# XThomasBU/video-gen-evals

Hardware: AMD Instinct MI355X
Metric: videos/sec scored (AC+TC) @32 frames/clip, 1/2/4/8 MI355X; |Δscore| vs ref (higher is better)
Workload: dtype f32x3; 1 GPU; BASELINE config 2: fusion-encoder fwd + AC/TC metrics, 256 clips x 32 frames per GPU, pre-extracted features resident in HBM (featurise included in the step); clips_per_gpu=256, frames_per_clip=32, windows_per_encode=256, parallelism=video-sharded x1

## Files before the change

video-gen-evals_amd/csrc/vge_encoder_x3s.hip:

```cpp
#include "vge_x3.h"
#include <type_traits>

#ifdef VGE_TRACE
__device__ long long g_x3s_trace[64 * 8 * 128];
#define XTS(k)                                                                                                       \
  do {                                                                                                              \
    if (tr_on && blockIdx.x < 64 && (threadIdx.x & 63) == 0)                                                        \
      g_x3s_trace[(blockIdx.x * 8 + (threadIdx.x >> 6)) * 128 + (k)] = __builtin_amdgcn_s_memtime();                 \
  } while (0)
#else
#define XTS(k) \
  do {         \
  } while (0)
#endif

namespace {

using vge::EncDescX3;

#ifndef X3S_TRACE_ROUND
#define X3S_TRACE_ROUND 0
#endif
#ifndef X3S_GELU
#define X3S_GELU 1
#endif
#ifndef X3S_PRIO
#define X3S_PRIO 1
#endif
constexpr int X3S_WMAX = 4;
#ifndef X3S_PF_QUAD
#define X3S_PF_QUAD 4
#endif
#ifndef X3S_PF_PAIR
#define X3S_PF_PAIR 8
#endif
#ifndef X3S_PF16_QUAD
#define X3S_PF16_QUAD 8
#endif
#ifndef X3S_PF16_PAIR
#define X3S_PF16_PAIR 8
#endif
#ifndef X3S_ROT
#define X3S_ROT 0
#endif
#ifndef X3S_SKIP
#define X3S_SKIP 1
#endif
constexpr int XR = 536;
constexpr int XRB = 2 * XR;
constexpr int XLO = 528;
template <int W>
constexpr int x3s_g() { return 32 / W; }
template <int W>
constexpr int x3s_wsb() { return 32 * XRB + (W >= 4 ? 128 : 0); }
template <int W>
constexpr int x3s_zr() { return W * x3s_wsb<W>(); }
template <int W>
__host__ __device__ constexpr int x3s_rwin(int r) { return ((r & 3) + 8 * (r >> 2)) / x3s_g<W>(); }
template <int W>
__host__ __device__ constexpr int x3s_rfr0(int t, int r) {
  return x3s_g<W>() * t + ((r & 3) + 8 * (r >> 2)) % x3s_g<W>();
}
template <int W, bool SKIP>
__device__ __forceinline__ bool x3s_tap_ok(int t, int o) {
  constexpr int G = x3s_g<W>();
  return !(X3S_SKIP && SKIP) || (G * t + G - 1 + o >= 0 && G * t + o <= 31);
}
constexpr int X3S_AUX_OFF = (x3s_zr<X3S_WMAX>() + XRB + 15) / 16 * 16;

struct X3sAux {
  int rexp[2][32 * X3S_WMAX];
  float stats[2][X3S_WMAX][8][2];
  float mx[2][2][X3S_WMAX][4];
  int ex[2][2][X3S_WMAX];
  int cnt[2];
};
constexpr int X3S_PRE_WAVE = 32 * 64 + 256;
constexpr int X3S_PRE_OFF = (X3S_AUX_OFF + (int)sizeof(X3sAux) + 15) / 16 * 16;
constexpr int X3S_LDS_BYTES = X3S_PRE_OFF + 8 * X3S_PRE_WAVE;
static_assert(X3S_AUX_OFF % 16 == 0, "aux alignment");
static_assert(X3S_LDS_BYTES <= 160 * 1024, "LDS");

template <int W, bool SKIP, bool SP>
__device__ __forceinline__ void stream_part(Acc<W, 1>& acc, const char* wb, int ntap, unsigned loff, const char* xa,
                                            int i, int dil, int ctr, int rot) {
  constexpr int R = W, G = x3s_g<W>();
  constexpr int PF = SP ? (R >= 4 ? X3S_PF_QUAD : X3S_PF_PAIR) : (R >= 4 ? X3S_PF16_QUAD : X3S_PF16_PAIR);
  static_assert(8 % PF == 0, "ring depth must divide a tap's 8 chunks");
  const char* xw = xa + (i / G) * x3s_wsb<W>();
  const int fi = i % G;
  const char* xz = xa + x3s_zr<W>();
  auto rowp = [&](int k, int t) -> const char* {
    const int tt = G * t + fi + (k - ctr) * dil;
    return (unsigned)tt < 32u ? xw + tt * XRB : xz;
  };
  const __amdgpu_buffer_rsrc_t rs =
      __builtin_amdgcn_make_buffer_rsrc(const_cast<char*>(wb), (short)0, 0x7FFFFFF0, 0x00020000);
  const unsigned loff_l = loff + PLANE_B;
  auto ldb = [&](int k, int j, BFrag<1>& b) {
    const int so = (k * 16 + ((j + rot) & 7)) * CHUNK_B;
    b.h[0] = __builtin_bit_cast(half8, __builtin_amdgcn_raw_buffer_load_b128(rs, loff, so, 0));
    if constexpr (SP) b.l[0] = __builtin_bit_cast(half8, __builtin_amdgcn_raw_buffer_load_b128(rs, loff_l, so, 0));
  };
  BFrag<1> b[PF];
#pragma unroll
  for (int j = 0; j < PF - 1; ++j) ldb(0, j, b[j]);
  half8 ah[R], al[R];
  const char* pt[R];
  bool okc[R];
#pragma unroll
  for (int t = 0; t < R; ++t) {
    pt[t] = rowp(0, t);
    okc[t] = x3s_tap_ok<W, SKIP>(t, -ctr * dil);
    if (okc[t]) {
      ah[t] = *reinterpret_cast<const half8*>(pt[t] + rot * 32);
      if constexpr (SP) al[t] = *reinterpret_cast<const half8*>(pt[t] + rot * 32 + XLO);
    }
  }
  for (int k = 0; k < ntap; ++k) {
    const bool more = k + 1 < ntap;
    const int kn = more ? k + 1 : k;
    const char* pn[R];
    bool okn[R];
#pragma unroll
    for (int t = 0; t < R; ++t) {
      pn[t] = rowp(kn, t);
      okn[t] = x3s_tap_ok<W, SKIP>(t, (kn - ctr) * dil);
    }
#pragma unroll
    for (int j = 0; j < 8; ++j) {
#if !(VGE_ABL & 2)
      if (j + PF - 1 < 8) ldb(k, j + PF - 1, b[(j + PF - 1) % PF]);
      else ldb(kn, more ? j + PF - 1 - 8 : 7, b[(j + PF - 1) % PF]);
#endif
#pragma unroll
      for (int t = 0; t < R; ++t) {
#if !(VGE_ABL & 1)
        if (okc[t]) {
          acc.c[t][0] = mfma32(ah[t], b[j % PF].h[0], acc.c[t][0]);
          if constexpr (SP) {
            acc.c[t][0] = mfma32(ah[t], b[j % PF].l[0], acc.c[t][0]);
            acc.c[t][0] = mfma32(al[t], b[j % PF].h[0], acc.c[t][0]);
          }
        }
#endif
#if !(VGE_ABL & 4)
        if (j < 7 ? okc[t] : okn[t]) {
          const char* q = j < 7 ? pt[t] + ((j + 1 + rot) & 7) * 32 : pn[t] + rot * 32;
          ah[t] = *reinterpret_cast<const half8*>(q);
          if constexpr (SP) al[t] = *reinterpret_cast<const half8*>(q + XLO);
        }
#endif
        __builtin_amdgcn_sched_barrier(0);
      }
      asm volatile("" ::: "memory");
    }
#pragma unroll
    for (int t = 0; t < R; ++t) {
      pt[t] = pn[t];
      okc[t] = okn[t];
    }
  }
}

__device__ __forceinline__ float gload(const float* p) {
  return *(const __attribute__((address_space(1))) float*)p;
}

template <int W, bool SP>
__device__ __forceinline__ void conv_x3s_body(const float* __restrict__ feats, int n_windows, int win0,
                                              const EncDescX3& ed, int e, float* __restrict__ enc_out, char* lds_raw,
                                              int& n_ex, int* __restrict__ status, int spin_limit,
                                              [[maybe_unused]] bool tr_on) {
  constexpr int R = W, G = x3s_g<W>(), WSB = x3s_wsb<W>();
  _Float16* X = reinterpret_cast<_Float16*>(lds_raw);
  char* Xb = lds_raw;
  X3sAux& ax = *reinterpret_cast<X3sAux*>(lds_raw + X3S_AUX_OFF);

  const int tid = threadIdx.x;
  const int wave = __builtin_amdgcn_readfirstlane(tid >> 6);
  const int grp = wave >> 2, wg = wave & 3;
  int lane, i, h, col;
  unsigned loff;
  const char* xa;
  auto lane_setup = [&]() {
    int t = tid;
    asm volatile("" : "+v"(t));
    lane = t & 63;
    i = lane & 31;
    h = lane >> 5;
    col = wave * 32 + i;
    loff = (unsigned)((h * 256 + col) * 16);
    xa = reinterpret_cast<const char*>(X) + h * 16;
  };
  lane_setup();
  auto crow = [&](int t, int r) { return x3s_rwin<W>(r) * 32 + x3s_rfr0<W>(t, r) + 4 * h; };
  auto cofs = [&](int t, int r) { return x3s_rwin<W>(r) * WSB + x3s_rfr0<W>(t, r) * XRB; };

  Acc<R, 1> acc;
  floatx16 res[R];
  for (int c = tid; c < XR; c += 512)
    *reinterpret_cast<_Float16*>(Xb + x3s_zr<W>() + 2 * c) = (_Float16)0.0f;

  auto afn_stem = [&](int c, AFrag<R>& f) {
#pragma unroll
    for (int t = 0; t < R; ++t) {
      const char* q = xa + (i / G) * WSB + (G * t + i % G) * XRB + c * 32;
      f.h[t] = *reinterpret_cast<const half8*>(q);
      if constexpr (SP) f.l[t] = *reinterpret_cast<const half8*>(q + XLO);
    }
  };
  XTS(0);
  acc.zero();
  constexpr int RPW = 32 * W / 8;
  constexpr int PG = W <= 2 ? 2 : 1;
  for (int p0 = 0; p0 < ed.n_stem_panels; p0 += PG) {
    float a[PG][RPW][4];
#pragma unroll
    for (int q = 0; q < PG; ++q) {
      const int p = p0 + q;
      const int kw = p < ed.n_stem_panels ? min(256, ed.d_in - p * 256) : 0;
#pragma unroll
      for (int jr = 0; jr < RPW; ++jr) {
        const int r = wave * RPW + jr;
        const int w = win0 + (r >> 5);
        const float* src = feats + ((size_t)w * VGE_T + (r & 31)) * ed.ld + ed.in_col + p * 256;
#pragma unroll
        for (int jc = 0; jc < 4; ++jc) {
          const int c = lane + 64 * jc;
          a[q][jr][jc] = (c < kw && w < n_windows) ? gload(src + c) : 0.f;
        }
      }
    }
#pragma unroll
    for (int q = 0; q < PG; ++q) {
      const int p = p0 + q;
      if (p >= ed.n_stem_panels) break;
      const int kw = min(256, ed.d_in - p * 256);
      int* ecur = ax.rexp[p & 1];
#pragma unroll
      for (int jr = 0; jr < RPW; ++jr) {
        float m = fmaxf(fmaxf(fabsf(a[q][jr][0]), fabsf(a[q][jr][1])), fmaxf(fabsf(a[q][jr][2]), fabsf(a[q][jr][3])));
        m = wave_max_all(m);
        const int ex = fp16_range_exp(m);
        const int r = wave * RPW + jr;
        if (lane == 0) ecur[r] = ex;
        _Float16* xr = reinterpret_cast<_Float16*>(Xb + (r >> 5) * WSB + (r & 31) * XRB);
#pragma unroll
        for (int jc = 0; jc < 4; ++jc) {
          const int c = lane + 64 * jc;
          if constexpr (SP) split_store(xr + c, xr + XLO / 2 + c, ldexpf(a[q][jr][jc], -ex));
          else xr[c] = (_Float16)ldexpf(a[q][jr][jc], -ex);
        }
      }
      __syncthreads();
      if (p == 0) XTS(122);
      if (p > 0) {
        const int* eprev = ax.rexp[(p - 1) & 1];
#pragma unroll
        for (int t = 0; t < R; ++t)
#pragma unroll
          for (int r = 0; r < 16; ++r) acc.c[t][0][r] *= ldexpf(1.0f, eprev[crow(t, r)] - ecur[crow(t, r)]);
      }
      run_stream<SP ? CONV_PF : CONV_PF16, SP>(acc, reinterpret_cast<const char*>(ed.stem) + (size_t)p * 16 * CHUNK_B,
                                ((kw + 127) >> 7) * STREAM_GROUP, loff, afn_stem);
      if (p == 0) XTS(123);
      __syncthreads();
    }
  }

  auto group_max = [&](float (&m)[R]) {
    const int par = n_ex & 1;
#pragma unroll
    for (int t = 0; t < R; ++t) {
      const float w = wave_max_last(m[t]);
      if (lane == 63) ax.mx[par][grp][t][wg] = w;
    }
    ++n_ex;
    if (lane == 63) __hip_atomic_fetch_add(&ax.cnt[grp], 1, __ATOMIC_RELEASE, __HIP_MEMORY_SCOPE_WORKGROUP);
    int spin = 0;
    for (; spin < spin_limit && __builtin_amdgcn_readfirstlane(__hip_atomic_load(
                                    &ax.cnt[grp], __ATOMIC_ACQUIRE, __HIP_MEMORY_SCOPE_WORKGROUP)) < 4 * n_ex;
         ++spin)
      __builtin_amdgcn_s_sleep(1);
    if (spin >= spin_limit &&
        __builtin_amdgcn_readfirstlane(__hip_atomic_load(&ax.cnt[grp], __ATOMIC_ACQUIRE, __HIP_MEMORY_SCOPE_WORKGROUP)) <
            4 * n_ex &&
        lane == 0)
      __hip_atomic_store(status, 1, __ATOMIC_RELAXED, __HIP_MEMORY_SCOPE_SYSTEM);
#pragma unroll
    for (int t = 0; t < R; ++t)
      m[t] = fmaxf(fmaxf(ax.mx[par][grp][t][0], ax.mx[par][grp][t][1]),
                   fmaxf(ax.mx[par][grp][t][2], ax.mx[par][grp][t][3]));
  };
  [[maybe_unused]] int tslot = 64;
  auto store_act = [&](auto get, int par) {
    XTS(tslot + 1);
    float m[R];
#pragma unroll
    for (int v = 0; v < R; ++v) m[v] = 0.f;
#pragma unroll
    for (int t = 0; t < R; ++t) {
      const floatx16& x = get(t);
#pragma unroll
      for (int r = 0; r < 16; ++r) m[x3s_rwin<W>(r)] = fmaxf(m[x3s_rwin<W>(r)], fabsf(x[r]));
    }
    group_max(m);
    XTS(tslot + 2);
    float scv[R];
#pragma unroll
    for (int v = 0; v < R; ++v) {
      const int ex = fp16_range_exp(m[v]);
      if (wg == 0 && lane == 0) ax.ex[par][grp][v] = ex;
      scv[v] = ldexpf(1.0f, -ex);
    }
    char* bh = Xb + (4 * h * XR + col) * 2;
#pragma unroll
    for (int t = 0; t < R; ++t) {
      const floatx16& x = get(t);
#pragma unroll
      for (int r = 0; r < 16; ++r) {
        const float y = x[r] * scv[x3s_rwin<W>(r)];
        const _Float16 hi = (_Float16)y;
        const int off = cofs(t, r);
        *reinterpret_cast<_Float16*>(bh + off) = hi;
        if constexpr (SP) *reinterpret_cast<_Float16*>(bh + XLO + off) = (_Float16)(y - (float)hi);
      }
    }
    XTS(tslot + 3);
    tslot += 4;
  };
  auto gn_stats = [&](int b, int t, float& mu, float& rstd) {
    const float(*s)[2] = ax.stats[b & 1][t];
    const float m = (((s[0][0] + s[1][0]) + (s[2][0] + s[3][0])) + ((s[4][0] + s[5][0]) + (s[6][0] + s[7][0]))) * 0.125f;
    float q = 0.f, d = 0.f;
#pragma unroll
    for (int w = 0; w < 8; ++w) {
      q += s[w][1];
      const float dm = s[w][0] - m;
      d = fmaf(dm, dm, d);
    }
    mu = m;
    rstd = 1.0f / sqrtf(fmaf(d, 1024.0f, q) * (1.0f / 8192.0f) + 1e-5f);
  };
  auto gelu_tile = [&](floatx16& v) {
    float y[16];
#pragma unroll
    for (int k = 0; k < 16; ++k) y[k] = v[k];
#if X3S_GELU
    gelu_fast_s(y);
#else
    gelu_many_s(y);
#endif
#pragma unroll
    for (int k = 0; k < 16; ++k) v[k] = y[k];
  };

  auto stem_epilogue = [&]() {
    XTS(tslot);
    const int* efin = ax.rexp[(ed.n_stem_panels - 1) & 1];
    const float wcs = gload(ed.cs + col);
#pragma unroll
    for (int t = 0; t < R; ++t) {
#pragma unroll
      for (int r = 0; r < 16; ++r) res[t][r] = ldexpf(acc.c[t][0][r] * wcs, efin[crow(t, r)]);
    }
    store_act([&](int t) -> const floatx16& { return res[t]; }, 0);
  };

  float pre_wcs = 0.f, pre_sx = 0.f, pre_sy = 0.f;
  char* pre_lds = lds_raw + X3S_PRE_OFF + wave * X3S_PRE_WAVE;
  auto prefetch = [&](auto kind_tag, int gi) {
    constexpr int KIND = decltype(kind_tag)::value;
    const int blk = gi >> 1;
    pre_wcs = gload(ed.cs + (1 + gi) * 256 + col);
    if constexpr (KIND == 2) {
      pre_sx = gload(ed.fold + 3 * 256 * 16 + col * 2);
      pre_sy = gload(ed.fold + 3 * 256 * 16 + col * 2 + 1);
    } else if constexpr (KIND == 0) {
      if (blk > 0) {
        const float* fb = ed.fold + ((size_t)(blk - 1) * 256 + wave * 32) * 16;
        glds16(fb + lane * 4, pre_lds);
        glds16(fb + 256 + lane * 4, pre_lds + 1024);
        const float* gsrc = (h ? ed.gn_b : ed.gn_w) + (blk - 1) * 256 + col;
        __builtin_amdgcn_global_load_lds((const __attribute__((address_space(1))) void*)gsrc,
                                         (__attribute__((address_space(3))) void*)(pre_lds + 2048), 4, 0, 0);
        asm volatile("" ::: "memory");
      }
    }
  };

  auto epilogue = [&](auto kind_tag, int gi) {
    constexpr int KIND = decltype(kind_tag)::value;
    XTS(tslot);
    const int par = gi & 1, blk = gi >> 1;
    const float wcs = pre_wcs;
    float scv[R];
#pragma unroll
    for (int v = 0; v < R; ++v) scv[v] = ldexpf(1.0f, ax.ex[par][1][v]) * wcs;
    if constexpr (KIND == 2) {
      const float2 sp = {pre_sx, pre_sy};
      float* ob = enc_out + (size_t)e * n_windows * VGE_T * VGE_D + col;
#pragma unroll
      for (int v = 0; v < R; ++v) {
        float mu, rstd;
        gn_stats(3, v, mu, rstd);
        const int win = win0 + v;
        if (win < n_windows) {
#pragma unroll
          for (int t = 0; t < R; ++t)
#pragma unroll
            for (int r = 0; r < 16; ++r)
              if (x3s_rwin<W>(r) == v)
                ob[((size_t)win * VGE_T + x3s_rfr0<W>(t, r) + 4 * h) * VGE_D] =
                    fmaf(rstd, fmaf(acc.c[t][0][r], scv[v], -mu * sp.x), sp.y);
        }
      }
    } else {
      constexpr int GH = G / 2;
      float cg[16], cb[16], gsv[R], gshv[R], muv[R], rstdv[R];
      if constexpr (KIND == 0) {
        if (blk > 0) {
          const int dil = 1 << blk;
          vmcnt0();
          const char* pl = pre_lds + i * 64;
          const floatx4 pre_g = *reinterpret_cast<const floatx4*>(pl);
          const float pre_g4 = *reinterpret_cast<const float*>(pl + 16);
          const floatx4 pre_b = *reinterpret_cast<const floatx4*>(pl + 32);
          const float pre_b4 = *reinterpret_cast<const float*>(pl + 48);
          const float pre_gw = *reinterpret_cast<const float*>(pre_lds + 2048 + i * 4);
          const float pre_gb = *reinterpret_cast<const float*>(pre_lds + 2048 + 128 + i * 4);
#pragma unroll
          for (int f = 0; f < 16; ++f) {
            const int row = x3s_rfr0<W>(f / GH, f % GH) + 4 * h;
            const bool k0 = row >= 2 * dil, k1 = row >= dil, k3 = row < 32 - dil, k4 = row < 32 - 2 * dil;
            cg[f] = (((k0 ? pre_g.x : 0.f) + (k1 ? pre_g.y : 0.f)) + pre_g.z) + (k3 ? pre_g.w : 0.f) + (k4 ? pre_g4 : 0.f);
            cb[f] = (((k0 ? pre_b.x : 0.f) + (k1 ? pre_b.y : 0.f)) + pre_b.z) + (k3 ? pre_b.w : 0.f) + (k4 ? pre_b4 : 0.f);
          }
#pragma unroll
          for (int v = 0; v < R; ++v) {
            gn_stats(blk - 1, v, muv[v], rstdv[v]);
            gsv[v] = rstdv[v] * pre_gw;
            gshv[v] = fmaf(-muv[v], gsv[v], pre_gb);
          }
        }
      }
#pragma unroll
      for (int t = 0; t < R; ++t) {
        floatx16& x = acc.c[t][0];
        if constexpr (KIND == 0) {
          if (blk > 0) {
#pragma unroll
            for (int r = 0; r < 16; ++r) {
              const int v = x3s_rwin<W>(r), f = t * GH + r % GH;
              res[t][r] = fmaf(res[t][r], gsv[v], gshv[v]);
              x[r] = fmaf(rstdv[v], fmaf(-muv[v], cg[f], x[r] * scv[v]), cb[f]);
            }
          } else {
#pragma unroll
            for (int r = 0; r < 16; ++r) x[r] *= scv[x3s_rwin<W>(r)];
          }
          gelu_tile(x);
        } else {
#pragma unroll
          for (int r = 0; r < 16; ++r) x[r] = fmaf(x[r], scv[x3s_rwin<W>(r)], res[t][r]);
          gelu_tile(x);
          res[t] = x;
        }
        __builtin_amdgcn_sched_barrier(0);
      }
      if constexpr (KIND == 1) {
        float mw[R], q[R];
#pragma unroll
        for (int v = 0; v < R; ++v) mw[v] = q[v] = 0.f;
#pragma unroll
        for (int t = 0; t < R; ++t)
#pragma unroll
          for (int r = 0; r < 16; ++r) mw[x3s_rwin<W>(r)] += res[t][r];
#pragma unroll
        for (int v = 0; v < R; ++v) {
          mw[v] = wave_sum_last(mw[v]);
          mw[v] = __builtin_bit_cast(float, __builtin_amdgcn_readlane(__builtin_bit_cast(int, mw[v]), 63)) *
                  (1.0f / 1024.0f);
        }
#pragma unroll
        for (int t = 0; t < R; ++t)
#pragma unroll
          for (int r = 0; r < 16; ++r) {
            const float d = res[t][r] - mw[x3s_rwin<W>(r)];
            q[x3s_rwin<W>(r)] = fmaf(d, d, q[x3s_rwin<W>(r)]);
          }
#pragma unroll
        for (int v = 0; v < R; ++v) q[v] = wave_sum_last(q[v]);
        if (lane == 63) {
#pragma unroll
          for (int v = 0; v < R; ++v) {
            ax.stats[blk & 1][v][wave][0] = mw[v];
            ax.stats[blk & 1][v][wave][1] = q[v];
          }
        }
      }
      store_act([&](int t) -> const floatx16& { return acc.c[t][0]; }, (gi + 1) & 1);
    }
  };

  auto stream = [&](auto skip_tag, int gi, int part) {
    constexpr bool SKIP = decltype(skip_tag)::value;
    if (part == 0) {
      acc.zero();
    } else {
      float f[R];
#pragma unroll
      for (int v = 0; v < R; ++v) f[v] = ldexpf(1.0f, ax.ex[gi & 1][0][v] - ax.ex[gi & 1][1][v]);
#pragma unroll
      for (int t = 0; t < R; ++t)
#pragma unroll
        for (int r = 0; r < 16; ++r) acc.c[t][0][r] *= f[x3s_rwin<W>(r)];
    }
    const bool proj = gi == 8;
    const char* wb = reinterpret_cast<const char*>(proj ? ed.proj : ed.conv + (size_t)gi * 80 * (CHUNK_B / 2)) +
                     (size_t)part * 8 * CHUNK_B;
    if (X3S_PRIO) __builtin_amdgcn_s_setprio(1);
    stream_part<W, SKIP, SP>(acc, wb, proj ? 1 : 5, loff, xa + part * 8 * 32, i, proj ? 0 : 1 << (gi >> 1),
                             proj ? 0 : 2, X3S_ROT ? __builtin_amdgcn_readfirstlane((int)(blockIdx.x >> 3) & 7) : 0);
    __builtin_amdgcn_s_setprio(0);
  };

  using K0 = std::integral_constant<int, 0>;
  using K1 = std::integral_constant<int, 1>;
  using K2 = std::integral_constant<int, 2>;
  [[maybe_unused]] int ph = 0;
  auto phase_end = [&]() {
    XTS(2 + 2 * ph);
    lds_barrier();
    XTS(3 + 2 * ph);
    ++ph;
    lane_setup();
  };
  XTS(1);
  if (grp == 1) phase_end();
  else lane_setup();
  stem_epilogue();
  phase_end();
  using NoSkip = std::integral_constant<bool, false>;
  using Skip = std::integral_constant<bool, true>;
  auto block = [&](auto skip_tag, int blk) {
    stream(skip_tag, 2 * blk, 0);
    phase_end();
    prefetch(K0{}, 2 * blk);
    stream(skip_tag, 2 * blk, 1);
    phase_end();
    epilogue(K0{}, 2 * blk);
    phase_end();
    stream(skip_tag, 2 * blk + 1, 0);
    phase_end();
    prefetch(K1{}, 2 * blk + 1);
    stream(skip_tag, 2 * blk + 1, 1);
    phase_end();
    epilogue(K1{}, 2 * blk + 1);
    phase_end();
  };
#pragma unroll 1
  for (int blk = 0; blk < 2; ++blk) block(NoSkip{}, blk);
#pragma unroll 1
  for (int blk = 2; blk < 4; ++blk) block(Skip{}, blk);
  stream(NoSkip{}, 8, 0);
  phase_end();
  prefetch(K2{}, 8);
  stream(NoSkip{}, 8, 1);
  phase_end();
  epilogue(K2{}, 8);
  phase_end();
  if (grp == 0) phase_end();
}

template <bool SP>
__global__ void __launch_bounds__(512, 1) conv_encoder_x3s_kernel(const float* __restrict__ feats,
                                                                   const EncDescX3* __restrict__ encs, vge::ConvSched cs,
                                                                   float* __restrict__ enc_out, int* __restrict__ status,
                                                                   int spin_limit) {
  extern __shared__ __attribute__((aligned(16))) char lds_raw[];
  X3sAux& ax = *reinterpret_cast<X3sAux*>(lds_raw + X3S_AUX_OFF);
  if (threadIdx.x < 2) ax.cnt[threadIdx.x] = 0;
#ifdef VGE_TRACE
  if (blockIdx.x < 64 && (threadIdx.x & 63) == 0)
    g_x3s_trace[(blockIdx.x * 8 + (threadIdx.x >> 6)) * 128 + 120] = __builtin_amdgcn_s_memtime();
#endif
  int n_ex = 0;
  const int n = cs.n_windows;
  const int bp = xcd_remap(blockIdx.x, cs.G);
#ifndef VGE_X3S_ROT
#define VGE_X3S_ROT 4
#endif
#ifndef VGE_X3S_ROT_BIT
#define VGE_X3S_ROT_BIT 0
#endif
#if VGE_X3S_ROT == 3
  const int rot = cs.n_units == 3 * cs.G ? bp % 3 : 0;
#elif VGE_X3S_ROT == 4
  const int rot = cs.G % 8 == 0 ? (bp / (cs.G / 8)) % ((cs.n_units + cs.G - 1) / cs.G) : 0;
#else
  const int rot = (VGE_X3S_ROT && cs.n_units == 3 * cs.G && ((bp >> VGE_X3S_ROT_BIT) & 1)) ? VGE_X3S_ROT : 0;
#endif
  const int n_rounds = (cs.n_units + cs.G - 1) / cs.G;
  for (int k = 0; k < n_rounds; ++k) {
    const int round = rot ? (k + rot) % n_rounds : k;
    const int u = round * cs.G + bp;
    if (u >= cs.n_units) continue;
    if (u < cs.Q) {
      int e, w0;
      conv_unit(cs, u, e, w0);
      conv_x3s_body<4, SP>(feats, n, w0, encs[e], e, enc_out, lds_raw, n_ex, status, spin_limit,
                       round == X3S_TRACE_ROUND);
    } else {
      int e, w0;
      conv_unit(cs, u, e, w0);
      conv_x3s_body<2, SP>(feats, n, w0, encs[e], e, enc_out, lds_raw, n_ex, status, spin_limit,
                       round == X3S_TRACE_ROUND);
    }
  }
#ifdef VGE_TRACE
  if (blockIdx.x < 64 && (threadIdx.x & 63) == 0)
    g_x3s_trace[(blockIdx.x * 8 + (threadIdx.x >> 6)) * 128 + 121] = __builtin_amdgcn_s_memtime();
#endif
}

}

namespace vge {

hipError_t encoder_x3s_kernel_setup() {
  hipError_t e = hipFuncSetAttribute((const void*)conv_encoder_x3s_kernel<true>,
                                     hipFuncAttributeMaxDynamicSharedMemorySize, X3S_LDS_BYTES);
  if (e == hipSuccess)
    e = hipFuncSetAttribute((const void*)conv_encoder_x3s_kernel<false>, hipFuncAttributeMaxDynamicSharedMemorySize,
                            X3S_LDS_BYTES);
  return e;
}

static int g_x3s_spin_limit = 1 << 22;

hipError_t launch_conv_encoders_x3s(const float* feats, int n_windows, const EncDescX3* encs, int n_enc, unsigned heavy,
                                    float* enc_out, int* status, bool split, hipStream_t s) {
  if (n_windows < 1 || n_enc < 1) return hipSuccess;
  if (!status) return hipErrorInvalidValue;
  const ConvSched cs = conv_quad_sched(n_windows, n_enc, heavy);
  if (split)
    hipLaunchKernelGGL(conv_encoder_x3s_kernel<true>, dim3(cs.G), dim3(512), X3S_LDS_BYTES, s, feats, encs, cs, enc_out,
                       status, g_x3s_spin_limit);
  else
    hipLaunchKernelGGL(conv_encoder_x3s_kernel<false>, dim3(cs.G), dim3(512), X3S_LDS_BYTES, s, feats, encs, cs, enc_out,
                       status, g_x3s_spin_limit);
  return hipGetLastError();
}

}

extern "C" int vge_debug_set_x3s_spin_limit(int n) {
  const int prev = vge::g_x3s_spin_limit;
  vge::g_x3s_spin_limit = n < 0 ? (1 << 22) : n;
  return prev;
}

#ifdef VGE_TRACE
extern "C" int vge_debug_x3s_trace(long long* host, int n) {
  return (int)hipMemcpyFromSymbol(host, HIP_SYMBOL(g_x3s_trace), sizeof(long long) * (size_t)n);
}
#endif
```

Before: 193,700 videos/s.

## Prime weight ring across barriers and carry prefetch between stream parts

The weight-fragment ring is hoisted out of stream_part into the kernel. Its first loads are now issued before each phase barrier, and at the end of part 0 the ring carries over into part 1 instead of being drained and reloaded. The fold and GroupNorm prefetch moves earlier, into the previous block's epilogue, and LDS pointers are typed address_space(3) so the compiler emits ds reads instead of flat loads. The aim is to hide global weight-load latency behind barriers and epilogues, at the cost of keeping more registers live across barriers.

```diff
diff --git a/video-gen-evals_amd/csrc/vge_encoder_x3s.hip b/video-gen-evals_amd/csrc/vge_encoder_x3s.hip
--- a/video-gen-evals_amd/csrc/vge_encoder_x3s.hip
+++ b/video-gen-evals_amd/csrc/vge_encoder_x3s.hip
@@ -81,46 +81,64 @@
 static_assert(X3S_AUX_OFF % 16 == 0, "aux alignment");
 static_assert(X3S_LDS_BYTES <= 160 * 1024, "LDS");
 
-template <int W, bool SKIP, bool SP>
-__device__ __forceinline__ void stream_part(Acc<W, 1>& acc, const char* wb, int ntap, unsigned loff, const char* xa,
-                                            int i, int dil, int ctr, int rot) {
+typedef const __attribute__((address_space(3))) char* lchar;
+typedef const __attribute__((address_space(3))) half8* lhalf8;
+
+template <int W, bool SP>
+constexpr int x3s_pf() {
+  return SP ? (W >= 4 ? X3S_PF_QUAD : X3S_PF_PAIR) : (W >= 4 ? X3S_PF16_QUAD : X3S_PF16_PAIR);
+}
+
+__device__ __forceinline__ __amdgpu_buffer_rsrc_t x3s_wrsrc(const char* wb) {
+  return __builtin_amdgcn_make_buffer_rsrc(const_cast<char*>(wb), (short)0, 0x7FFFFFF0, 0x00020000);
+}
+template <bool SP>
+__device__ __forceinline__ void x3s_ldb(__amdgpu_buffer_rsrc_t rs, unsigned loff, int chunk, BFrag<1>& b) {
+  const int so = chunk * CHUNK_B;
+  b.h[0] = __builtin_bit_cast(half8, __builtin_amdgcn_raw_buffer_load_b128(rs, loff, so, 0));
+  if constexpr (SP) b.l[0] = __builtin_bit_cast(half8, __builtin_amdgcn_raw_buffer_load_b128(rs, loff + PLANE_B, so, 0));
+}
+
+template <int W, bool SP, int PF>
+__device__ __forceinline__ void prime_part(BFrag<1> (&b)[PF], const char* wb, unsigned loff, int rot) {
+  static_assert(PF == x3s_pf<W, SP>(), "the caller's ring has this unit's depth");
+  const __amdgpu_buffer_rsrc_t rs = x3s_wrsrc(wb);
+#pragma unroll
+  for (int j = 0; j < PF - 1; ++j) x3s_ldb<SP>(rs, loff, (j + rot) & 7, b[j]);
+}
+
+template <int W, bool SKIP, bool SP, bool CARRY, int PF>
+__device__ __forceinline__ void stream_part(Acc<W, 1>& acc, BFrag<1> (&b)[PF], const char* wb, int ntap,
+                                            unsigned loff, const char* xa, int i, int dil, int ctr, int rot) {
   constexpr int R = W, G = x3s_g<W>();
-  constexpr int PF = SP ? (R >= 4 ? X3S_PF_QUAD : X3S_PF_PAIR) : (R >= 4 ? X3S_PF16_QUAD : X3S_PF16_PAIR);
+  static_assert(PF == x3s_pf<W, SP>(), "the caller's ring has this unit's depth");
   static_assert(8 % PF == 0, "ring depth must divide a tap's 8 chunks");
-  const char* xw = xa + (i / G) * x3s_wsb<W>();
+  const lchar xl = (lchar)xa;
+  const lchar xw = xl + (i / G) * x3s_wsb<W>();
   const int fi = i % G;
-  const char* xz = xa + x3s_zr<W>();
-  auto rowp = [&](int k, int t) -> const char* {
+  const lchar xz = xl + x3s_zr<W>();
+  auto rowp = [&](int k, int t) -> lchar {
     const int tt = G * t + fi + (k - ctr) * dil;
     return (unsigned)tt < 32u ? xw + tt * XRB : xz;
   };
-  const __amdgpu_buffer_rsrc_t rs =
-      __builtin_amdgcn_make_buffer_rsrc(const_cast<char*>(wb), (short)0, 0x7FFFFFF0, 0x00020000);
-  const unsigned loff_l = loff + PLANE_B;
-  auto ldb = [&](int k, int j, BFrag<1>& b) {
-    const int so = (k * 16 + ((j + rot) & 7)) * CHUNK_B;
-    b.h[0] = __builtin_bit_cast(half8, __builtin_amdgcn_raw_buffer_load_b128(rs, loff, so, 0));
-    if constexpr (SP) b.l[0] = __builtin_bit_cast(half8, __builtin_amdgcn_raw_buffer_load_b128(rs, loff_l, so, 0));
-  };
-  BFrag<1> b[PF];
-#pragma unroll
-  for (int j = 0; j < PF - 1; ++j) ldb(0, j, b[j]);
+  const __amdgpu_buffer_rsrc_t rs = x3s_wrsrc(wb);
+  auto ldb = [&](int k, int j, BFrag<1>& f) { x3s_ldb<SP>(rs, loff, k * 16 + ((j + rot) & 7), f); };
   half8 ah[R], al[R];
-  const char* pt[R];
+  lchar pt[R];
   bool okc[R];
 #pragma unroll
   for (int t = 0; t < R; ++t) {
     pt[t] = rowp(0, t);
     okc[t] = x3s_tap_ok<W, SKIP>(t, -ctr * dil);
     if (okc[t]) {
-      ah[t] = *reinterpret_cast<const half8*>(pt[t] + rot * 32);
-      if constexpr (SP) al[t] = *reinterpret_cast<const half8*>(pt[t] + rot * 32 + XLO);
+      ah[t] = *reinterpret_cast<lhalf8>(pt[t] + rot * 32);
+      if constexpr (SP) al[t] = *reinterpret_cast<lhalf8>(pt[t] + rot * 32 + XLO);
     }
   }
   for (int k = 0; k < ntap; ++k) {
     const bool more = k + 1 < ntap;
     const int kn = more ? k + 1 : k;
-    const char* pn[R];
+    lchar pn[R];
     bool okn[R];
 #pragma unroll
     for (int t = 0; t < R; ++t) {
@@ -131,7 +149,10 @@
     for (int j = 0; j < 8; ++j) {
 #if !(VGE_ABL & 2)
       if (j + PF - 1 < 8) ldb(k, j + PF - 1, b[(j + PF - 1) % PF]);
-      else ldb(kn, more ? j + PF - 1 - 8 : 7, b[(j + PF - 1) % PF]);
+      else {
+        const int jn = (j + PF - 1 - 8 + rot) & 7;
+        x3s_ldb<SP>(rs, loff, more ? (k + 1) * 16 + jn : CARRY ? 8 + jn : k * 16 + ((7 + rot) & 7), b[(j + PF - 1) % PF]);
+      }
 #endif
 #pragma unroll
       for (int t = 0; t < R; ++t) {
@@ -146,9 +167,9 @@
 #endif
 #if !(VGE_ABL & 4)
         if (j < 7 ? okc[t] : okn[t]) {
-          const char* q = j < 7 ? pt[t] + ((j + 1 + rot) & 7) * 32 : pn[t] + rot * 32;
-          ah[t] = *reinterpret_cast<const half8*>(q);
-          if constexpr (SP) al[t] = *reinterpret_cast<const half8*>(q + XLO);
+          const lchar q = j < 7 ? pt[t] + ((j + 1 + rot) & 7) * 32 : pn[t] + rot * 32;
+          ah[t] = *reinterpret_cast<lhalf8>(q);
+          if constexpr (SP) al[t] = *reinterpret_cast<lhalf8>(q + XLO);
         }
 #endif
         __builtin_amdgcn_sched_barrier(0);
@@ -372,22 +393,22 @@
   char* pre_lds = lds_raw + X3S_PRE_OFF + wave * X3S_PRE_WAVE;
   auto prefetch = [&](auto kind_tag, int gi) {
     constexpr int KIND = decltype(kind_tag)::value;
-    const int blk = gi >> 1;
     pre_wcs = gload(ed.cs + (1 + gi) * 256 + col);
     if constexpr (KIND == 2) {
       pre_sx = gload(ed.fold + 3 * 256 * 16 + col * 2);
       pre_sy = gload(ed.fold + 3 * 256 * 16 + col * 2 + 1);
-    } else if constexpr (KIND == 0) {
-      if (blk > 0) {
-        const float* fb = ed.fold + ((size_t)(blk - 1) * 256 + wave * 32) * 16;
-        glds16(fb + lane * 4, pre_lds);
-        glds16(fb + 256 + lane * 4, pre_lds + 1024);
-        const float* gsrc = (h ? ed.gn_b : ed.gn_w) + (blk - 1) * 256 + col;
-        __builtin_amdgcn_global_load_lds((const __attribute__((address_space(1))) void*)gsrc,
-                                         (__attribute__((address_space(3))) void*)(pre_lds + 2048), 4, 0, 0);
-        asm volatile("" ::: "memory");
-      }
-    }
+    }
+  };
+  auto prefetch_fold = [&](int blk) {
+    const float* fb = ed.fold + ((size_t)(blk - 1) * 256 + wave * 32) * 16;
+    glds16(fb + lane * 4, pre_lds);
+    glds16(fb + 256 + lane * 4, pre_lds + 1024);
+    const float *gw = ed.gn_w, *gb = ed.gn_b;
+    asm volatile("" : "+s"(gw), "+s"(gb));
+    const float* gsrc = (h ? gb : gw) + (blk - 1) * 256 + col;
+    __builtin_amdgcn_global_load_lds((const __attribute__((address_space(1))) void*)gsrc,
+                                     (__attribute__((address_space(3))) void*)(pre_lds + 2048), 4, 0, 0);
+    asm volatile("" ::: "memory");
   };
 
   auto epilogue = [&](auto kind_tag, int gi) {
@@ -504,9 +525,24 @@
     }
   };
 
-  auto stream = [&](auto skip_tag, int gi, int part) {
+  BFrag<1> ring[x3s_pf<W, SP>()];
+  const int crot = X3S_ROT ? __builtin_amdgcn_readfirstlane((int)(blockIdx.x >> 3) & 7) : 0;
+  auto wpart = [&](int gi, int part) {
+    return reinterpret_cast<const char*>(gi == 8 ? ed.proj : ed.conv + (size_t)gi * 80 * (CHUNK_B / 2)) +
+           (size_t)part * 8 * CHUNK_B;
+  };
+  auto prime = [&](int gi) { prime_part<W, SP>(ring, wpart(gi, 0), loff, crot); };
+  auto ring_landed = [&]() {
+#pragma unroll
+    for (int j = 0; j < x3s_pf<W, SP>() - 1; ++j) {
+      asm volatile("" : "+v"(ring[j].h[0]));
+      if constexpr (SP) asm volatile("" : "+v"(ring[j].l[0]));
+    }
+  };
+  auto stream = [&](auto skip_tag, int gi, auto part_tag) {
     constexpr bool SKIP = decltype(skip_tag)::value;
-    if (part == 0) {
+    constexpr int part = decltype(part_tag)::value;
+    if constexpr (part == 0) {
       acc.zero();
     } else {
       float f[R];
@@ -518,11 +554,9 @@
         for (int r = 0; r < 16; ++r) acc.c[t][0][r] *= f[x3s_rwin<W>(r)];
     }
     const bool proj = gi == 8;
-    const char* wb = reinterpret_cast<const char*>(proj ? ed.proj : ed.conv + (size_t)gi * 80 * (CHUNK_B / 2)) +
-                     (size_t)part * 8 * CHUNK_B;
     if (X3S_PRIO) __builtin_amdgcn_s_setprio(1);
-    stream_part<W, SKIP, SP>(acc, wb, proj ? 1 : 5, loff, xa + part * 8 * 32, i, proj ? 0 : 1 << (gi >> 1),
-                             proj ? 0 : 2, X3S_ROT ? __builtin_amdgcn_readfirstlane((int)(blockIdx.x >> 3) & 7) : 0);
+    stream_part<W, SKIP, SP, part == 0>(acc, ring, wpart(gi, part), proj ? 1 : 5, loff, xa + part * 8 * 32, i,
+                                        proj ? 0 : 1 << (gi >> 1), proj ? 0 : 2, crot);
     __builtin_amdgcn_s_setprio(0);
   };
 
@@ -541,33 +575,41 @@
   if (grp == 1) phase_end();
   else lane_setup();
   stem_epilogue();
+  prime(0);
   phase_end();
   using NoSkip = std::integral_constant<bool, false>;
   using Skip = std::integral_constant<bool, true>;
+  using P0 = std::integral_constant<int, 0>;
+  using P1 = std::integral_constant<int, 1>;
   auto block = [&](auto skip_tag, int blk) {
-    stream(skip_tag, 2 * blk, 0);
+    ring_landed();
+    stream(skip_tag, 2 * blk, P0{});
     phase_end();
     prefetch(K0{}, 2 * blk);
-    stream(skip_tag, 2 * blk, 1);
+    stream(skip_tag, 2 * blk, P1{});
     phase_end();
     epilogue(K0{}, 2 * blk);
+    prime(2 * blk + 1);
     phase_end();
-    stream(skip_tag, 2 * blk + 1, 0);
+    stream(skip_tag, 2 * blk + 1, P0{});
     phase_end();
     prefetch(K1{}, 2 * blk + 1);
-    stream(skip_tag, 2 * blk + 1, 1);
+    stream(skip_tag, 2 * blk + 1, P1{});
     phase_end();
     epilogue(K1{}, 2 * blk + 1);
+    if (blk < 3) prefetch_fold(blk + 1);
+    prime(2 * blk + 2);
     phase_end();
   };
 #pragma unroll 1
   for (int blk = 0; blk < 2; ++blk) block(NoSkip{}, blk);
 #pragma unroll 1
   for (int blk = 2; blk < 4; ++blk) block(Skip{}, blk);
-  stream(NoSkip{}, 8, 0);
+  ring_landed();
+  stream(NoSkip{}, 8, P0{});
   phase_end();
   prefetch(K2{}, 8);
-  stream(NoSkip{}, 8, 1);
+  stream(NoSkip{}, 8, P1{});
   phase_end();
   epilogue(K2{}, 8);
   phase_end();
```

Result: faster. 195,900 videos/s (median of 6 runs) (+1.1%).
